# hmorimitsu/ptlflow

Measured on AMD Instinct MI355X. Metric: frame-pairs/sec, RAFT 32-iter 436x1024, higher is better.
Workload: dtype f32; 1 GPU; raft random-init (seeded), 436x1024 frame pairs, 32 iterations, fp32, batch 8/GPU, eval forward incl. encoders, mask head + convex upsample on every iteration as the reference; global_batch=8, parallelism=dp1 (independent replicas, no collectives)

## Files before the change

ptlflow_amd/csrc/pfk_wino.hip:

```cpp
#include "pfk_gemm.h"

using namespace pfkg;

namespace {

constexpr int WT = 32;
constexpr int WN = 64;
constexpr int WK = 8;
constexpr int UIMG = 16 * WN * WK;

typedef float f32x2 __attribute__((ext_vector_type(2)));
typedef __attribute__((address_space(3))) float lfloat;
typedef __attribute__((address_space(3))) f32x2 lf32x2;
typedef __attribute__((address_space(3))) f32x4 lf32x4;

struct WinoArgs {
  const float* src; int ld;
  unsigned src_bytes;
  int H, W;
  int tw, tpi;
  int ntiles;
  int nks;
  const float* weight; unsigned w_bytes;
  const float* bias;
  int cout;
  int ncb;
  int relu; float scale;
  float* out; int out_ld, out_coff;
  unsigned out_bytes;
  const float* res; int res_ld;
  unsigned res_bytes;
  int relu2;
  int vec;
  const float* in_mean; const float* in_rstd;
  unsigned stat_bytes;
  int cin, in_relu;
  int nbi;
  double* part; long long astride;
};

constexpr unsigned T_OK = 0x80000000u, T_ROW2 = 0x40000000u, T_COL2 = 0x20000000u, T_PIX = 0x1fffffffu;
constexpr int ESZ = 64 * 32 + 4 * 16;

__device__ __forceinline__ __amdgpu_buffer_rsrc_t rsrc_n(const void* p, unsigned bytes) {
  return __builtin_amdgcn_make_buffer_rsrc(const_cast<void*>(p), 0, (int)bytes, 0x00020000);
}

__device__ __forceinline__ void wino_load_stat(__amdgpu_buffer_rsrc_t rm, __amdgpu_buffer_rsrc_t rr, unsigned soff, int ks, float (&mr)[2]) {
  mr[0] = __builtin_bit_cast(float, __builtin_amdgcn_raw_buffer_load_b32(rm, soff, ks * WK * 4, 0));
  mr[1] = __builtin_bit_cast(float, __builtin_amdgcn_raw_buffer_load_b32(rr, soff, ks * WK * 4, 0));
}

__device__ __forceinline__ void wino_load_v2(__amdgpu_buffer_rsrc_t rs, const unsigned (&voff)[16], int ks, int q, float (&d)[16]) {
  d[q] = __builtin_bit_cast(float, __builtin_amdgcn_raw_buffer_load_b32(rs, voff[q], ks * WK * 4, 0));
  d[q + 1] = __builtin_bit_cast(float, __builtin_amdgcn_raw_buffer_load_b32(rs, voff[q + 1], ks * WK * 4, 0));
}

__device__ __forceinline__ void wino_dma_u(__amdgpu_buffer_rsrc_t rw, lfloat* dst, unsigned wvoff, unsigned wk, int j) {
#if defined(__HIP_DEVICE_COMPILE__)
  __builtin_amdgcn_raw_ptr_buffer_load_lds(rw, (__attribute__((address_space(3))) void*)(dst + j * 1024), 16, wvoff, wk + j * 4096u, 0, 0);
#endif
}

template <bool NORM>
__device__ __forceinline__ void wino_mfma(const lfloat* aV, const lfloat* aU, const lfloat* aU1, f32x4 (&acc)[16][2], bool more,
                                          __amdgpu_buffer_rsrc_t rw, lfloat* udst, unsigned wvoff, unsigned wk,
                                          __amdgpu_buffer_rsrc_t rs, const unsigned (&voff)[16], int ks, float (&d)[16],
                                          __amdgpu_buffer_rsrc_t rm, __amdgpu_buffer_rsrc_t rr, unsigned soff, float (&mr)[2]) {
  f32x2 va[2], u0[2], u1[2];
  va[0] = *(const lf32x2*)(aV);
  u0[0] = *(const lf32x2*)(aU);
  u1[0] = *(const lf32x2*)(aU1);
  __builtin_amdgcn_sched_barrier(0);
#pragma unroll
  for (int x = 0; x < 16; ++x) {
    const int c = x & 1, n = c ^ 1;
    if (x + 1 < 16) {
      va[n] = *(const lf32x2*)(aV + (x + 1) * WT * WK);
      u0[n] = *(const lf32x2*)(aU + (x + 1) * WN * WK);
      u1[n] = *(const lf32x2*)(aU1 + (x + 1) * WN * WK);
    }
    if (more) {
      if (x < 8) wino_dma_u(rw, udst, wvoff, wk, x);
      else wino_load_v2(rs, voff, ks, 2 * (x - 8), d);
      if constexpr (NORM) {
        if (x == 8) wino_load_stat(rm, rr, soff, ks, mr);
      }
    }
    __builtin_amdgcn_sched_barrier(0);
    acc[x][0] = __builtin_amdgcn_mfma_f32_16x16x4f32(va[c][0], u0[c][0], acc[x][0], 0, 0, 0);
    acc[x][1] = __builtin_amdgcn_mfma_f32_16x16x4f32(va[c][0], u1[c][0], acc[x][1], 0, 0, 0);
    acc[x][0] = __builtin_amdgcn_mfma_f32_16x16x4f32(va[c][1], u0[c][1], acc[x][0], 0, 0, 0);
    acc[x][1] = __builtin_amdgcn_mfma_f32_16x16x4f32(va[c][1], u1[c][1], acc[x][1], 0, 0, 0);
    __builtin_amdgcn_sched_barrier(0);
  }
}

typedef __attribute__((address_space(3))) unsigned lunsigned;
typedef unsigned int u32x4v __attribute__((__vector_size__(16)));

template <bool RES, bool VEC>
__device__ __forceinline__ void wino_epi_request(const WinoArgs& a, const lunsigned* tT, int n0, unsigned (&oo)[8], f32x4 (&r4)[8]) {
  unsigned ro[8];
#pragma unroll
  for (int i = 0; i < 8; ++i) {
    oo[i] = tT[2 * i] + (unsigned)(a.out_coff + n0) * 4u;
    if constexpr (RES) ro[i] = tT[4 * WT + 2 * i] + (unsigned)n0 * 4u;
  }
  if constexpr (RES) {
    const __amdgpu_buffer_rsrc_t rr = rsrc_n(a.res, a.res_bytes);
#pragma unroll
    for (int i = 0; i < 8; ++i) {
      if constexpr (VEC) {
        r4[i] = __builtin_bit_cast(f32x4, __builtin_amdgcn_raw_buffer_load_b128(rr, ro[i], 0, 0));
      } else {
#pragma unroll
        for (int j = 0; j < 4; ++j)
          r4[i][j] = __builtin_bit_cast(float, __builtin_amdgcn_raw_buffer_load_b32(rr, n0 + j < a.cout ? ro[i] + 4u * j : OOB, 0, 0));
      }
    }
  }
}

template <bool RES, bool VEC, bool STATS>
__device__ __forceinline__ void wino_epi_store(const WinoArgs& a, const lfloat* rE, int n0, const unsigned (&oo)[8], const f32x4 (&r4)[8],
                                               double (&st)[8]) {
  const __amdgpu_buffer_rsrc_t ro = rsrc_n(a.out, a.out_bytes);
  const __amdgpu_buffer_rsrc_t rbias = rsrc_n(a.bias, a.bias != nullptr ? (unsigned)a.cout * 4u : 0u);
  float bias4[4];
#pragma unroll
  for (int j = 0; j < 4; ++j) bias4[j] = __builtin_bit_cast(float, __builtin_amdgcn_raw_buffer_load_b32(rbias, (unsigned)(n0 + j) * 4u, 0, 0));
  const float lo = a.relu ? 0.f : -__builtin_inff(), lo2 = a.relu2 ? 0.f : -__builtin_inff();
#pragma unroll
  for (int i = 0; i < 8; ++i) {
    const f32x4 y = *(const lf32x4*)(rE + i * 256 + (i >> 1) * 16);
    float v[4];
#pragma unroll
    for (int j = 0; j < 4; ++j) {
      float t = y[j] + bias4[j];
      t = (t < lo) ? lo : t;
      if constexpr (RES) {
        t = __builtin_fmaf(t, a.scale, r4[i][j]);
        t = (t < lo2) ? lo2 : t;
      } else {
        t *= a.scale;
      }
      v[j] = t;
      if constexpr (STATS) {
        const double dv = (double)((oo[i] < OOB && (VEC || n0 + j < a.cout)) ? t : 0.f);
        st[j] += dv;
        st[4 + j] = __builtin_fma(dv, dv, st[4 + j]);
      }
    }
    if constexpr (VEC) {
      __builtin_amdgcn_raw_buffer_store_b128(__builtin_bit_cast(u32x4v, (f32x4{v[0], v[1], v[2], v[3]})), ro, oo[i], 0, 0);
    } else {
#pragma unroll
      for (int j = 0; j < 4; ++j)
        __builtin_amdgcn_raw_buffer_store_b32(__builtin_bit_cast(unsigned, v[j]), ro, n0 + j < a.cout ? oo[i] + 4u * j : OOB, 0, 0);
    }
  }
}

template <bool RES, bool NORM = false, bool STATS = false>
__global__ __launch_bounds__(256, 2) void conv_gemm_wino_f32_kernel(const WinoArgs a) {
  static_assert(!(RES && STATS), "the residual form is never in front of an instance norm");
  __shared__ __attribute__((aligned(16))) float smem[2 * UIMG + 16 * WT * WK];
  lfloat* const sU = (lfloat*)smem;
  lfloat* const sV = sU + 2 * UIMG;

  const int tid = threadIdx.x, lane = tid & 63, wid = __builtin_amdgcn_readfirstlane(tid >> 6);
  const int cb = blockIdx.x % a.ncb;
  const int t0 = (blockIdx.x / a.ncb) * WT;

  const __amdgpu_buffer_rsrc_t rs = rsrc_n(a.src, a.src_bytes);
  const __amdgpu_buffer_rsrc_t rw = rsrc_n(a.weight, a.w_bytes);
  const __amdgpu_buffer_rsrc_t rm = rsrc_n(a.in_mean, NORM ? a.stat_bytes : 0u);
  const __amdgpu_buffer_rsrc_t rr = rsrc_n(a.in_rstd, NORM ? a.stat_bytes : 0u);

  const int lt = tid >> 3, cc = tid & 7;
  unsigned voff[16];
  unsigned tinfo;
  unsigned soff = 0;
  {
    int g, b, r;
    bool tok;
    if constexpr (STATS) {
      const int tb = blockIdx.x / a.ncb;
      b = tb / a.nbi;
      r = (tb - b * a.nbi) * WT + lt;
      tok = r < a.tpi;
    } else {
      g = t0 + lt;
      tok = g < a.ntiles;
      b = g / a.tpi;
      r = g - b * a.tpi;
    }
    if constexpr (NORM) soff = ((unsigned)b * (unsigned)a.cin + (unsigned)cc) * 4u;
    const int ty = r / a.tw, tx = r - ty * a.tw;
    tinfo = tok ? (T_OK | (2 * ty + 1 < a.H ? T_ROW2 : 0u) | (2 * tx + 1 < a.W ? T_COL2 : 0u) | (unsigned)((b * a.H + 2 * ty) * a.W + 2 * tx)) : 0u;
#pragma unroll
    for (int i = 0; i < 4; ++i)
#pragma unroll
      for (int j = 0; j < 4; ++j) {
        const int y = 2 * ty - 1 + i, x = 2 * tx - 1 + j;
        const bool ok = tok && (unsigned)y < (unsigned)a.H && (unsigned)x < (unsigned)a.W;
        voff[i * 4 + j] = ok ? ((unsigned)((b * a.H + y) * a.W + x) * (unsigned)a.ld + (unsigned)cc) * 4u : OOB;
      }
  }
  const int vslot = ((cc & 3) * 2 + (cc >> 2)) ^ (((lt >> 2) & 3) * 2);
  lfloat* const vdst = sV + lt * WK + vslot;
  const unsigned wvoff = (unsigned)lane * 16u;
  const unsigned wbase = (unsigned)cb * (unsigned)a.nks * (UIMG * 4u) + (unsigned)wid * 1024u;
  lfloat* const udst = sU + wid * 256;

  float d[16];
  float mr[2] = {0.f, 0.f};
  const int wt = wid & 1, wc = wid >> 1;
  const int rl = lane & 15, kq = lane >> 4;
  const lfloat* const aV = sV + (wt * 16 + rl) * WK + ((kq * 2) ^ (((rl >> 2) & 3) * 2));
  const lfloat* const aU = sU + (wc * 32 + rl) * WK + ((kq * 2) ^ (((rl >> 2) & 3) * 2));
  const lfloat* aU1 = aU + 16 * WK;
  asm volatile("" : "+v"(aU1));

  f32x4 acc[16][2];
#pragma unroll
  for (int x = 0; x < 16; ++x)
#pragma unroll
    for (int c = 0; c < 2; ++c) acc[x][c] = f32x4{0.f, 0.f, 0.f, 0.f};

#pragma unroll
  for (int j = 0; j < 8; ++j) {
    wino_dma_u(rw, udst, wvoff, wbase, j);
    wino_load_v2(rs, voff, 0, 2 * j, d);
  }
  if constexpr (NORM) wino_load_stat(rm, rr, soff, 0, mr);
  const float nlo = a.in_relu ? 0.f : -__builtin_inff();  for (int ks = 0; ks < a.nks; ++ks) {
    if constexpr (NORM) {
#pragma unroll
      for (int q = 0; q < 16; ++q) {
        const float y = __fmul_rn(__fsub_rn(d[q], mr[0]), mr[1]);
        d[q] = voff[q] == OOB ? 0.f : ((y < nlo) ? nlo : y);
      }
    }
    float t[16];
#pragma unroll
    for (int j = 0; j < 4; ++j) {
      t[0 * 4 + j] = d[0 * 4 + j] - d[2 * 4 + j];
      t[1 * 4 + j] = d[1 * 4 + j] + d[2 * 4 + j];
      t[2 * 4 + j] = d[2 * 4 + j] - d[1 * 4 + j];
      t[3 * 4 + j] = d[1 * 4 + j] - d[3 * 4 + j];
    }
#pragma unroll
    for (int i = 0; i < 4; ++i) {
      vdst[(i * 4 + 0) * WT * WK] = t[i * 4 + 0] - t[i * 4 + 2];
      vdst[(i * 4 + 1) * WT * WK] = t[i * 4 + 1] + t[i * 4 + 2];
      vdst[(i * 4 + 2) * WT * WK] = t[i * 4 + 2] - t[i * 4 + 1];
      vdst[(i * 4 + 3) * WT * WK] = t[i * 4 + 1] - t[i * 4 + 3];
    }
    asm volatile("s_waitcnt vmcnt(0) lgkmcnt(0)\n\ts_barrier" ::: "memory");
    const int ub = (ks & 1) * UIMG;
    wino_mfma<NORM>(aV, aU + ub, aU1 + ub, acc, ks + 1 < a.nks, rw, udst + (UIMG - ub), wvoff, wbase + (unsigned)(ks + 1) * (UIMG * 4u),
                    rs, voff, ks + 1, d, rm, rr, soff, mr);
    asm volatile("s_waitcnt lgkmcnt(0)\n\ts_barrier" ::: "memory");
  }

  lfloat* const sE = (lfloat*)smem + wid * ESZ;
  lunsigned* const sT = (lunsigned*)((lfloat*)smem + 4 * ESZ);
  static_assert(4 * ESZ + 8 * WT <= 2 * UIMG + 16 * WT * WK, "parking areas and offset table must fit into the loop's LDS");
  {
    const unsigned need = T_OK | ((cc & 2) ? T_ROW2 : 0u) | ((cc & 1) ? T_COL2 : 0u);
    const bool ok = (tinfo & need) == need;
    const unsigned pix = (tinfo & T_PIX) + (unsigned)(((cc >> 1) & 1) * a.W + (cc & 1));
    const unsigned po = ok ? pix * (unsigned)a.out_ld * 4u : OOB;
    const unsigned pr = ok ? pix * (unsigned)a.res_ld * 4u : OOB;
    if (cc < 4) {
      sT[cc * WT + lt] = po;
      if constexpr (RES) sT[(4 + cc) * WT + lt] = pr;
    }
  }
  asm volatile("s_waitcnt lgkmcnt(0)\n\ts_barrier" ::: "memory");

  const int prow = lane >> 3, c4 = (lane & 7) * 4;
  const int n0 = cb * WN + wc * 32 + c4;
  const lunsigned* const tT = sT + (prow & 3) * WT + wt * 16 + (lane >> 5);
  const bool vec = a.vec && cb * WN + wc * 32 + 32 <= a.cout;
  unsigned oo[8];
  f32x4 r4[8];
  if (vec) wino_epi_request<RES, true>(a, tT, n0, oo, r4);
  else wino_epi_request<RES, false>(a, tT, n0, oo, r4);

  {
    lfloat* const pE = sE + kq * (16 * 32 + 16) + rl;
#pragma unroll
    for (int c = 0; c < 2; ++c)
#pragma unroll
      for (int r = 0; r < 4; ++r) {
        float m[16];
#pragma unroll
        for (int x = 0; x < 16; ++x) m[x] = acc[x][c][r];
        float s0[4], s1[4];
#pragma unroll
        for (int j = 0; j < 4; ++j) {
          s0[j] = m[0 * 4 + j] + m[1 * 4 + j] + m[2 * 4 + j];
          s1[j] = m[1 * 4 + j] - m[2 * 4 + j] - m[3 * 4 + j];
        }
        pE[(r * 4 + 0) * 32 + c * 16] = s0[0] + s0[1] + s0[2];
        pE[(r * 4 + 1) * 32 + c * 16] = s0[1] - s0[2] - s0[3];
        pE[(r * 4 + 2) * 32 + c * 16] = s1[0] + s1[1] + s1[2];
        pE[(r * 4 + 3) * 32 + c * 16] = s1[1] - s1[2] - s1[3];
      }
  }
  const lfloat* const rE = sE + prow * 32 + c4;
  double st[8] = {0., 0., 0., 0., 0., 0., 0., 0.};
  if (vec) wino_epi_store<RES, true, STATS>(a, rE, n0, oo, r4, st);
  else wino_epi_store<RES, false, STATS>(a, rE, n0, oo, r4, st);

  if constexpr (STATS) {
    typedef __attribute__((address_space(3))) double ldouble;
    ldouble* const sS = (ldouble*)(sE) + lane * 8;
#pragma unroll
    for (int j = 0; j < 8; ++j) sS[j] = st[j];
    asm volatile("s_waitcnt lgkmcnt(0)\n\ts_barrier" ::: "memory");
    if (tid < 2 * WN) {
      const int which = tid >> 6, col = tid & 63;
      const int idx = ((col & 31) >> 2) * 8 + which * 4 + (col & 3);
      double tot[2];
#pragma unroll
      for (int w = 0; w < 2; ++w) {
        const ldouble* const p = (const ldouble*)((lfloat*)smem + ((col >> 5) * 2 + w) * ESZ) + idx;
        double s = 0.;
#pragma unroll
        for (int k = 0; k < 8; ++k) s += p[k * 64];
        tot[w] = s;
      }
      const int n = cb * WN + col;
      if (n < a.cout) a.part[which * a.astride + (long long)(blockIdx.x / a.ncb) * a.cout + n] = tot[0] + tot[1];
    }
  }
}

constexpr int WN1 = 128;
constexpr int VIMG1 = 8 * WT * WK;

struct Wino1dArgs {
  const float* src0; const float* src1;
  int ld0, ld1;
  unsigned bytes0, bytes1;
  int nks0, nks;
  int H, W;
  int L, nt;
  int ntiles;
  const float* weight; unsigned w_bytes;
  const float* bias;
  int cout, ncb;
  int relu; float scale;
  float* out; int out_ld, out_coff;
  const float* res; int res_ld;
  float* h; int h_ld;
  float* aux_z; float* aux_rh;
  int ch;
};

template <bool VERT>
__device__ __forceinline__ void wino1d_tile(const Wino1dArgs& a, int g, int& base, int& t) {
  if constexpr (VERT) {
    const int r = g / a.W, x = g - r * a.W, b = r / a.nt;
    t = r - b * a.nt;
    base = b * a.H * a.W + x;
  } else {
    const int line = g / a.nt;
    t = g - line * a.nt;
    base = line * a.W;
  }
}

__device__ __forceinline__ void wino1d_load_v(__amdgpu_buffer_rsrc_t rs0, __amdgpu_buffer_rsrc_t rs1, const unsigned (&voff0)[8],
                                              const unsigned (&voff1)[8], bool s1, int soff, int q, float (&d)[8]) {
  d[q] = s1 ? __builtin_bit_cast(float, __builtin_amdgcn_raw_buffer_load_b32(rs1, voff1[q], soff, 0))
            : __builtin_bit_cast(float, __builtin_amdgcn_raw_buffer_load_b32(rs0, voff0[q], soff, 0));
}

__device__ __forceinline__ void wino1d_mfma(const lfloat* aV, const lfloat* aU0, const lfloat* aU1, const lfloat* aU2, const lfloat* aU3,
                                            f32x4 (&acc)[8][4], bool more, __amdgpu_buffer_rsrc_t rw, lfloat* udst, unsigned wvoff,
                                            unsigned wk, __amdgpu_buffer_rsrc_t rs0, __amdgpu_buffer_rsrc_t rs1,
                                            const unsigned (&voff0)[8], const unsigned (&voff1)[8], bool s1, int soff, float (&d)[8]) {
  f32x2 va[2], u[2][4];
  va[0] = *(const lf32x2*)(aV);
  u[0][0] = *(const lf32x2*)(aU0);
  u[0][1] = *(const lf32x2*)(aU1);
  u[0][2] = *(const lf32x2*)(aU2);
  u[0][3] = *(const lf32x2*)(aU3);
  __builtin_amdgcn_sched_barrier(0);
#pragma unroll
  for (int x = 0; x < 8; ++x) {
    const int c = x & 1, n = c ^ 1;
    if (x + 1 < 8) {
      va[n] = *(const lf32x2*)(aV + (x + 1) * WT * WK);
      u[n][0] = *(const lf32x2*)(aU0 + (x + 1) * WN1 * WK);
      u[n][1] = *(const lf32x2*)(aU1 + (x + 1) * WN1 * WK);
      u[n][2] = *(const lf32x2*)(aU2 + (x + 1) * WN1 * WK);
      u[n][3] = *(const lf32x2*)(aU3 + (x + 1) * WN1 * WK);
    }
    if (more) {
      wino_dma_u(rw, udst, wvoff, wk, x);
      wino1d_load_v(rs0, rs1, voff0, voff1, s1, soff, x, d);
    }
    __builtin_amdgcn_sched_barrier(0);
#pragma unroll
    for (int s = 0; s < 2; ++s)
#pragma unroll
      for (int f = 0; f < 4; ++f) acc[x][f] = __builtin_amdgcn_mfma_f32_16x16x4f32(va[c][s], u[c][f][s], acc[x][f], 0, 0, 0);
    __builtin_amdgcn_sched_barrier(0);
  }
}

__device__ __forceinline__ void wino1d_at(const f32x4 (&acc)[8][4], int f, int r, float (&y)[4]) {
  const float p12 = acc[1][f][r] + acc[2][f][r], q12 = acc[1][f][r] - acc[2][f][r];
  const float p34 = acc[3][f][r] + acc[4][f][r], q34 = acc[3][f][r] - acc[4][f][r];
  const float p56 = acc[5][f][r] + acc[6][f][r], q56 = acc[5][f][r] - acc[6][f][r];
  y[0] = acc[0][f][r] + p12 + p34 + p56;
  y[1] = q12 + 2.f * q34 + 0.5f * q56;
  y[2] = p12 + 4.f * p34 + 0.25f * p56;
  y[3] = q12 + 8.f * q34 + 0.125f * q56 + acc[7][f][r];
}

template <bool VERT, int EPI>
__global__ __launch_bounds__(256, 2) void conv_gemm_wino1d_f32_kernel(const Wino1dArgs a) {
  __shared__ __attribute__((aligned(16))) float smem[2 * UIMG + VIMG1];
  lfloat* const sU = (lfloat*)smem;
  lfloat* const sV = sU + 2 * UIMG;

  const int tid = threadIdx.x, lane = tid & 63, wid = __builtin_amdgcn_readfirstlane(tid >> 6);
  const int cb = blockIdx.x % a.ncb;
  const int t0 = (blockIdx.x / a.ncb) * WT;
  const int pstride = VERT ? a.W : 1;

  const __amdgpu_buffer_rsrc_t rs0 = rsrc_n(a.src0, a.bytes0);
  const __amdgpu_buffer_rsrc_t rs1 = rsrc_n(a.src1, a.bytes1);
  const __amdgpu_buffer_rsrc_t rw = rsrc_n(a.weight, a.w_bytes);

  const int lt = tid >> 3, cc = tid & 7;
  unsigned voff0[8], voff1[8];
  {
    const int g = t0 + lt;
    const bool tok = g < a.ntiles;
    int base, t;
    wino1d_tile<VERT>(a, g, base, t);
#pragma unroll
    for (int j = 0; j < 8; ++j) {
      const int ax = 4 * t - 2 + j;
      const bool ok = tok && (unsigned)ax < (unsigned)a.L;
      const unsigned pix = (unsigned)(base + ax * pstride);
      voff0[j] = ok ? (pix * (unsigned)a.ld0 + (unsigned)cc) * 4u : OOB;
      voff1[j] = ok ? (pix * (unsigned)a.ld1 + (unsigned)cc) * 4u : OOB;
    }
  }
  const int vslot = ((cc & 3) * 2 + (cc >> 2)) ^ (((lt >> 2) & 3) * 2);
  lfloat* const vdst = sV + lt * WK + vslot;
  const unsigned wvoff = (unsigned)lane * 16u;
  const unsigned wbase = (unsigned)cb * (unsigned)a.nks * (UIMG * 4u) + (unsigned)wid * 1024u;
  lfloat* const udst = sU + wid * 256;

  float d[8];
  const int wt = wid & 1, wc = wid >> 1;
  const int rl = lane & 15, kq = lane >> 4;
  const int oslot = (kq * 2) ^ (((rl >> 2) & 3) * 2);
  const lfloat* const aV = sV + (wt * 16 + rl) * WK + oslot;
  const lfloat* const aU0 = sU + (wc * 64 + rl) * WK + oslot;
  const lfloat* aU1 = aU0 + 16 * WK;
  const lfloat* aU2 = aU0 + 32 * WK;
  const lfloat* aU3 = aU0 + 48 * WK;
  asm volatile("" : "+v"(aU1));
  asm volatile("" : "+v"(aU2));
  asm volatile("" : "+v"(aU3));

  f32x4 acc[8][4];
#pragma unroll
  for (int x = 0; x < 8; ++x)
#pragma unroll
    for (int f = 0; f < 4; ++f) acc[x][f] = f32x4{0.f, 0.f, 0.f, 0.f};

#pragma unroll
  for (int j = 0; j < 8; ++j) {
    wino_dma_u(rw, udst, wvoff, wbase, j);
    wino1d_load_v(rs0, rs1, voff0, voff1, false, 0, j, d);
  }
  for (int ks = 0; ks < a.nks; ++ks) {
    {
      const float e12 = d[2] - 4.25f * d[4] + d[6], o12 = d[1] - 4.25f * d[3] + d[5];
      const float e34 = 0.25f * d[2] - 1.25f * d[4] + d[6], o34 = 0.5f * d[1] - 2.5f * d[3] + 2.f * d[5];
      const float e56 = 4.f * d[2] - 5.f * d[4] + d[6], o56 = 2.f * d[1] - 2.5f * d[3] + 0.5f * d[5];
      vdst[0 * WT * WK] = (d[6] - d[0]) + 5.25f * (d[2] - d[4]);
      vdst[1 * WT * WK] = e12 + o12;
      vdst[2 * WT * WK] = e12 - o12;
      vdst[3 * WT * WK] = e34 + o34;
      vdst[4 * WT * WK] = e34 - o34;
      vdst[5 * WT * WK] = e56 + o56;
      vdst[6 * WT * WK] = e56 - o56;
      vdst[7 * WT * WK] = (d[7] - d[1]) + 5.25f * (d[3] - d[5]);
    }
    asm volatile("s_waitcnt vmcnt(0) lgkmcnt(0)\n\ts_barrier" ::: "memory");
    const int ub = (ks & 1) * UIMG;
    const int kn = ks + 1;
    const bool s1 = kn >= a.nks0;
    const int soff = (kn - (s1 ? a.nks0 : 0)) * WK * 4;
    wino1d_mfma(aV, aU0 + ub, aU1 + ub, aU2 + ub, aU3 + ub, acc, kn < a.nks, rw, udst + (UIMG - ub), wvoff,
                wbase + (unsigned)kn * (UIMG * 4u), rs0, rs1, voff0, voff1, s1, soff, d);
    asm volatile("s_waitcnt lgkmcnt(0)\n\ts_barrier" ::: "memory");
  }

  typedef __attribute__((address_space(1))) float gfloat;
  if constexpr (EPI == PFK_EPI_LINEAR) {
#pragma unroll
    for (int f = 0; f < 4; ++f) {
      const int n = cb * WN1 + wc * 64 + f * 16 + rl;
      const bool nok = n < a.cout;
      const float bias = (a.bias != nullptr && nok) ? a.bias[n] : 0.f;
#pragma unroll
      for (int r = 0; r < 4; ++r) {
        const int g = t0 + wt * 16 + kq * 4 + r;
        float y[4];
        wino1d_at(acc, f, r, y);
        if (!nok || g >= a.ntiles) continue;
        int base, t;
        wino1d_tile<VERT>(a, g, base, t);
#pragma unroll
        for (int e = 0; e < 4; ++e) {
          const int ax = 4 * t + e;
          if (ax >= a.L) continue;
          const long long p = base + ax * pstride;
          float v = y[e] + bias;
          if (a.relu) v = (v < 0.f) ? 0.f : v;
          v *= a.scale;
          ((gfloat*)a.out)[p * a.out_ld + a.out_coff + n] = v;
        }
      }
    }
  } else {
    constexpr int ES = 68;
    static_assert(4 * 64 * ES <= 2 * UIMG + VIMG1, "the four waves' parking areas must fit into the loop's LDS");
    lfloat* const sE = (lfloat*)smem + wid * (64 * ES);
#pragma unroll
    for (int f = 0; f < 4; ++f)
#pragma unroll
      for (int r = 0; r < 4; ++r) {
        float y[4];
        wino1d_at(acc, f, r, y);
#pragma unroll
        for (int e = 0; e < 4; ++e) sE[((kq * 4 + r) * 4 + e) * ES + f * 16 + rl] = y[e];
      }
    const int prow = lane >> 4, col4 = (lane & 15) * 4;
    const int n0 = cb * WN1 + wc * 64 + col4;
    const bool nok = n0 < a.cout;
    const int nc = nok ? n0 : 0;
    const int ch = a.ch;
    f32x4 bias4 = f32x4{0.f, 0.f, 0.f, 0.f};
    if (a.bias != nullptr) bias4 = f32x4{a.bias[nc], a.bias[nc + 1], a.bias[nc + 2], a.bias[nc + 3]};
    const bool upper = nc >= ch;
    const int hc = (EPI == PFK_EPI_GRU_ZR) ? (upper ? nc - ch : 0) : nc;
#pragma unroll
    for (int half = 0; half < 2; ++half) {
      bool ok[8];
      long long p[8];
      f32x4 r4[8], h4[8], z4[8];
#pragma unroll
      for (int i = 0; i < 8; ++i) {
        const int li = (half * 8 + i) * 4 + prow;
        const int g = t0 + wt * 16 + (li >> 2);
        int base, t;
        wino1d_tile<VERT>(a, g, base, t);
        const int ax = 4 * t + (li & 3);
        ok[i] = nok && g < a.ntiles && ax < a.L;
        p[i] = ok[i] ? base + ax * pstride : 0;
        r4[i] = f32x4{0.f, 0.f, 0.f, 0.f};
        if (a.res != nullptr) r4[i] = *(const f32x4*)(a.res + p[i] * a.res_ld + nc);
        if constexpr (EPI == PFK_EPI_GRU_ZR) {
          if (upper) h4[i] = *(const f32x4*)(a.h + p[i] * a.h_ld + hc);
        } else {
          z4[i] = *(const f32x4*)(a.aux_z + p[i] * ch + nc);
          h4[i] = *(const f32x4*)(a.h + p[i] * a.h_ld + hc);
        }
      }
#pragma unroll
      for (int i = 0; i < 8; ++i) {
        const int li = (half * 8 + i) * 4 + prow;
        const f32x4 v = *(const lf32x4*)(sE + li * ES + col4) + bias4 + r4[i];
        f32x4 o;
        if constexpr (EPI == PFK_EPI_GRU_ZR) {
#pragma unroll
          for (int e = 0; e < 4; ++e) o[e] = sigmoid_f(v[e]);
          if (!ok[i]) continue;
          if (upper) {
#pragma unroll
            for (int e = 0; e < 4; ++e) o[e] *= h4[i][e];
            *(f32x4*)(a.aux_rh + p[i] * ch + hc) = o;
          } else {
            *(f32x4*)(a.aux_z + p[i] * ch + nc) = o;
          }
        } else {
#pragma unroll
          for (int e = 0; e < 4; ++e) {
            const float keep = __fmul_rn(__fsub_rn(1.0f, z4[i][e]), h4[i][e]);
            const float take = __fmul_rn(z4[i][e], tanhf(v[e]));
            o[e] = __fadd_rn(keep, take);
          }
          if (!ok[i]) continue;
          *(f32x4*)(a.h + p[i] * a.h_ld + hc) = o;
        }
      }
    }
  }
}

template <bool VERT>
static void wino1d_launch_epi(const Wino1dArgs& a, int epilogue, unsigned nblk, hipStream_t st) {
  switch (epilogue) {
    case PFK_EPI_GRU_ZR: hipLaunchKernelGGL((conv_gemm_wino1d_f32_kernel<VERT, PFK_EPI_GRU_ZR>), dim3(nblk), dim3(256), 0, st, a); break;
    case PFK_EPI_GRU_Q: hipLaunchKernelGGL((conv_gemm_wino1d_f32_kernel<VERT, PFK_EPI_GRU_Q>), dim3(nblk), dim3(256), 0, st, a); break;
    default: hipLaunchKernelGGL((conv_gemm_wino1d_f32_kernel<VERT, PFK_EPI_LINEAR>), dim3(nblk), dim3(256), 0, st, a); break;
  }
}

}

extern "C" {

long long pfk_conv_wino1d_weight_floats(int ktot, int cout) {
  if (ktot <= 0 || cout <= 0 || (ktot & 7)) return PFK_ERR_BAD_ARG;
  return 8LL * ktot * ((cout + WN1 - 1) / WN1 * WN1);
}

int pfk_conv1d_wino_f32(const pfk_conv_desc* d, pfk_stream_t stream) {
  if (!d) return PFK_ERR_BAD_ARG;
  const bool vert = d->kh == 5 && d->kw == 1;
  if (!vert && !(d->kh == 1 && d->kw == 5)) return PFK_ERR_UNSUPPORTED;
  if (d->stride > 1 || d->num_src < 1 || d->num_src > 2 || d->relu_after_residual) return PFK_ERR_UNSUPPORTED;
  if (d->epilogue != PFK_EPI_LINEAR && d->epilogue != PFK_EPI_GRU_ZR && d->epilogue != PFK_EPI_GRU_Q) return PFK_ERR_UNSUPPORTED;
  if (d->cout_active > 0 && d->cout_active < d->cout) return PFK_ERR_UNSUPPORTED;
  if (d->epilogue == PFK_EPI_LINEAR && d->residual) return PFK_ERR_UNSUPPORTED;
  if (!d->weight || d->B <= 0 || d->H <= 0 || d->W <= 0 || d->cout <= 0) return PFK_ERR_BAD_ARG;
  const long long M = (long long)d->B * d->H * d->W;
  int ktot = 0;
  for (int i = 0; i < d->num_src; ++i) {
    const pfk_conv_src& s = d->src[i];
    if (!s.ptr || s.channels <= 0 || s.ld < s.channels) return PFK_ERR_BAD_ARG;
    if (s.channels & 7) return PFK_ERR_UNSUPPORTED;
    if (reinterpret_cast<uintptr_t>(s.ptr) & 3u) return PFK_ERR_ALIGNMENT;
    if (M * s.ld * 4 >= 0x7fffffffLL) return PFK_ERR_UNSUPPORTED;
    ktot += s.channels;
  }
  const int ch = d->epilogue == PFK_EPI_GRU_ZR ? d->cout / 2 : d->cout;
  if (d->epilogue == PFK_EPI_LINEAR) {
    if (!d->out || d->out_coff < 0 || d->out_ld < d->out_coff + d->cout) return PFK_ERR_BAD_ARG;
    if (reinterpret_cast<uintptr_t>(d->out) & 3u) return PFK_ERR_ALIGNMENT;
  } else {
    if (!d->h || !d->aux_z || d->h_ld < ch || (d->epilogue == PFK_EPI_GRU_ZR && (!d->aux_rh || (d->cout & 1))) || (ch & 3))
      return PFK_ERR_BAD_ARG;
    if (d->residual && d->residual_ld < d->cout) return PFK_ERR_BAD_ARG;
    if (!pfk_aligned16(d->h) || !pfk_aligned16(d->aux_z) || !pfk_aligned16(d->aux_rh) || !pfk_aligned16(d->residual) || (d->h_ld & 3) ||
        (d->residual && (d->residual_ld & 3)))
      return PFK_ERR_ALIGNMENT;
  }
  if (!pfk_aligned16(d->weight)) return PFK_ERR_ALIGNMENT;
  const long long wfloats = pfk_conv_wino1d_weight_floats(ktot, d->cout);
  if (wfloats * 4 >= 0x7fffffffLL) return PFK_ERR_UNSUPPORTED;
  Wino1dArgs a{};
  const pfk_conv_src& s0 = d->src[0];
  const pfk_conv_src& s1 = d->src[d->num_src - 1];
  a.src0 = s0.ptr; a.ld0 = s0.ld; a.bytes0 = (unsigned)(((M - 1) * s0.ld + s0.channels) * 4);
  a.src1 = s1.ptr; a.ld1 = s1.ld; a.bytes1 = (unsigned)(((M - 1) * s1.ld + s1.channels) * 4);
  a.nks0 = s0.channels / WK; a.nks = ktot / WK;
  a.H = d->H; a.W = d->W;
  a.L = vert ? d->H : d->W;
  a.nt = (a.L + 3) / 4;
  const long long ntiles = (long long)d->B * (vert ? d->W : d->H) * a.nt;
  a.ncb = (d->cout + WN1 - 1) / WN1;
  const long long nblk = (ntiles + WT - 1) / WT * a.ncb;
  if (nblk >= 0x7fffffffLL) return PFK_ERR_UNSUPPORTED;
  a.ntiles = (int)ntiles;
  a.weight = d->weight; a.w_bytes = (unsigned)(wfloats * 4);
  a.bias = d->bias;
  a.cout = d->cout;
  a.relu = d->relu ? 1 : 0; a.scale = d->scale;
  a.out = d->out; a.out_ld = d->out_ld; a.out_coff = d->out_coff;
  a.res = d->residual; a.res_ld = d->residual_ld;
  a.h = d->h; a.h_ld = d->h_ld; a.aux_z = d->aux_z; a.aux_rh = d->aux_rh; a.ch = ch;
  if (vert) wino1d_launch_epi<true>(a, d->epilogue, (unsigned)nblk, static_cast<hipStream_t>(stream));
  else wino1d_launch_epi<false>(a, d->epilogue, (unsigned)nblk, static_cast<hipStream_t>(stream));
  return pfk_launch_status();
}

long long pfk_conv_wino_weight_floats(int cin, int cout) {
  if (cin <= 0 || cout <= 0 || (cin & 31)) return PFK_ERR_BAD_ARG;
  return 16LL * cin * ((cout + WN - 1) / WN * WN);
}

static inline long long wino_blocks_per_image(int H, int W) { return ((long long)((H + 1) / 2) * ((W + 1) / 2) + WT - 1) / WT; }

struct WinoFuse {
  bool norm, stats;
  const float* in_mean; const float* in_rstd; int in_relu;
  float eps; float* out_mean; float* out_rstd; void* workspace; long long workspace_bytes;
};

static int wino_launch(const pfk_conv_desc* d, bool res, pfk_stream_t stream, const WinoFuse* f = nullptr) {
  if (!d) return PFK_ERR_BAD_ARG;
  const bool norm = f && f->norm, stats = f && f->stats;
  if (norm && (!f->in_mean || !f->in_rstd)) return PFK_ERR_BAD_ARG;
  if (stats && (!f->out_mean || !f->out_rstd || !f->workspace || d->residual || d->relu_after_residual)) return PFK_ERR_BAD_ARG;
  if (d->num_src != 1 || d->kh != 3 || d->kw != 3 || d->stride > 1 || d->epilogue != PFK_EPI_LINEAR)
    return PFK_ERR_UNSUPPORTED;
  if (!res && (d->residual || d->relu_after_residual)) return PFK_ERR_UNSUPPORTED;
  if (res && (!d->residual || d->residual_ld < d->cout || (reinterpret_cast<uintptr_t>(d->residual) & 3u))) return PFK_ERR_BAD_ARG;
  const pfk_conv_src& s = d->src[0];
  if (!s.ptr || !d->weight || !d->out || d->B <= 0 || d->H <= 0 || d->W <= 0 || d->cout <= 0 || s.channels <= 0 ||
      s.ld < s.channels || d->out_coff < 0 || d->out_ld < d->out_coff + d->cout)
    return PFK_ERR_BAD_ARG;
  if (s.channels & 31) return PFK_ERR_UNSUPPORTED;
  if (!pfk_aligned16(d->weight) || (reinterpret_cast<uintptr_t>(s.ptr) & 3u) || (reinterpret_cast<uintptr_t>(d->out) & 3u))
    return PFK_ERR_ALIGNMENT;
  const long long M = (long long)d->B * d->H * d->W;
  const long long src_bytes = ((M - 1) * s.ld + s.channels) * 4;
  const long long wfloats = pfk_conv_wino_weight_floats(s.channels, d->cout);
  if (M * s.ld * 4 >= 0x7fffffffLL || wfloats * 4 >= 0x7fffffffLL) return PFK_ERR_UNSUPPORTED;
  const long long out_bytes = ((M - 1) * d->out_ld + d->out_coff + d->cout) * 4;
  const long long res_bytes = res ? ((M - 1) * d->residual_ld + d->cout) * 4 : 0;
  if (out_bytes >= 0x7fffffffLL || res_bytes >= 0x7fffffffLL) return PFK_ERR_UNSUPPORTED;
  int ncb = (d->cout + WN - 1) / WN;
  if (d->cout_active > 0 && d->cout_active < d->cout) {
    if (d->cout_active & (WN - 1)) return PFK_ERR_UNSUPPORTED;
    ncb = d->cout_active / WN;
    if (stats) return PFK_ERR_UNSUPPORTED;
  }
  if (norm && ((reinterpret_cast<uintptr_t>(f->in_mean) | reinterpret_cast<uintptr_t>(f->in_rstd)) & 3u)) return PFK_ERR_ALIGNMENT;
  if (stats) {
    if (reinterpret_cast<uintptr_t>(f->workspace) & 7u) return PFK_ERR_ALIGNMENT;
    if (f->workspace_bytes < pfk_conv_wino_stats_workspace_bytes(d->B, d->H, d->W, d->cout)) return PFK_ERR_BAD_ARG;
  }
  WinoArgs a{};
  a.src = s.ptr; a.ld = s.ld; a.src_bytes = (unsigned)src_bytes;
  a.H = d->H; a.W = d->W;
  a.tw = (d->W + 1) / 2;
  a.tpi = a.tw * ((d->H + 1) / 2);
  const long long ntiles = (long long)d->B * a.tpi;
  const long long nbi = wino_blocks_per_image(d->H, d->W);
  const long long nblk = (stats ? d->B * nbi : (ntiles + WT - 1) / WT) * ncb;
  if (nblk >= 0x7fffffffLL || ntiles >= 0x7fffffffLL) return PFK_ERR_UNSUPPORTED;
  a.ntiles = (int)ntiles;
  a.nks = s.channels / WK;
  a.weight = d->weight; a.w_bytes = (unsigned)(wfloats * 4);
  a.bias = d->bias;
  a.cout = d->cout;
  a.ncb = ncb;
  a.relu = d->relu ? 1 : 0; a.scale = d->scale;
  a.out = d->out; a.out_ld = d->out_ld; a.out_coff = d->out_coff; a.out_bytes = (unsigned)out_bytes;
  a.vec = pfk_aligned16(d->out + d->out_coff) && !(d->out_ld & 3) && (!res || (pfk_aligned16(d->residual) && !(d->residual_ld & 3)));
  if (norm) {
    a.in_mean = f->in_mean; a.in_rstd = f->in_rstd; a.in_relu = f->in_relu ? 1 : 0;
    a.cin = s.channels; a.stat_bytes = (unsigned)((long long)d->B * s.channels * 4);
  }
  hipStream_t st = static_cast<hipStream_t>(stream);
  if (stats) {
    a.nbi = (int)nbi;
    a.part = static_cast<double*>(f->workspace);
    a.astride = (long long)d->B * nbi * d->cout;
    if (norm) hipLaunchKernelGGL((conv_gemm_wino_f32_kernel<false, true, true>), dim3((unsigned)nblk), dim3(256), 0, st, a);
    else hipLaunchKernelGGL((conv_gemm_wino_f32_kernel<false, false, true>), dim3((unsigned)nblk), dim3(256), 0, st, a);
    return pfk_instnorm_finish_parts(a.part, d->B, a.nbi, d->cout, d->H * d->W, f->eps, f->out_mean, f->out_rstd, st);
  }
  if (norm) {
    if (res) return PFK_ERR_UNSUPPORTED;
    hipLaunchKernelGGL((conv_gemm_wino_f32_kernel<false, true, false>), dim3((unsigned)nblk), dim3(256), 0, st, a);
    return pfk_launch_status();
  }
  if (res) {
    if (d->cout_active > 0 && d->cout_active < d->cout) return PFK_ERR_UNSUPPORTED;
    a.res = d->residual; a.res_ld = d->residual_ld; a.res_bytes = (unsigned)res_bytes; a.relu2 = d->relu_after_residual ? 1 : 0;
    hipLaunchKernelGGL(conv_gemm_wino_f32_kernel<true>, dim3((unsigned)nblk), dim3(256), 0, static_cast<hipStream_t>(stream), a);
  } else {
    hipLaunchKernelGGL(conv_gemm_wino_f32_kernel<false>, dim3((unsigned)nblk), dim3(256), 0, static_cast<hipStream_t>(stream), a);
  }
  return pfk_launch_status();
}

int pfk_conv2d_wino_f32(const pfk_conv_desc* d, pfk_stream_t stream) { return wino_launch(d, false, stream); }

int pfk_conv2d_wino_res_f32(const pfk_conv_desc* d, pfk_stream_t stream) { return wino_launch(d, true, stream); }

int pfk_conv2d_wino_norm_f32(const pfk_conv_desc* d, const float* in_mean, const float* in_rstd, int in_relu, pfk_stream_t stream) {
  const WinoFuse f{true, false, in_mean, in_rstd, in_relu, 0.f, nullptr, nullptr, nullptr, 0};
  return wino_launch(d, false, stream, &f);
}

long long pfk_conv_wino_stats_workspace_bytes(int B, int H, int W, int cout) {
  if (B <= 0 || H <= 0 || W <= 0 || cout <= 0) return PFK_ERR_BAD_ARG;
  return 2LL * B * wino_blocks_per_image(H, W) * cout * (long long)sizeof(double);
}

int pfk_conv2d_wino_stats_f32(const pfk_conv_desc* d, const float* in_mean, const float* in_rstd, int in_relu, float eps,
                              float* out_mean, float* out_rstd, void* workspace, long long workspace_bytes, pfk_stream_t stream) {
  if ((in_mean == nullptr) != (in_rstd == nullptr)) return PFK_ERR_BAD_ARG;
  const WinoFuse f{in_mean != nullptr, true, in_mean, in_rstd, in_relu, eps, out_mean, out_rstd, workspace, workspace_bytes};
  return wino_launch(d, false, stream, &f);
}


}
```

Measured before the change: 125.0 frame-pairs/s.

## Software-pipeline 1D Winograd conv: double-buffer V tile, prefetch input two K-steps ahead

Restructures the 1D Winograd conv main loop so the input transform for the next K-step runs inside the MFMA loop into a second V buffer. Global input loads are issued two steps ahead, with a partial vmcnt wait. This removes the serial transform-then-barrier phase before each MFMA block and leaves a single barrier per step. The cost is extra LDS for the second V image, possibly lowering occupancy, plus more register pressure from holding two input vectors.

```diff
diff --git a/ptlflow_amd/csrc/pfk_wino.hip b/ptlflow_amd/csrc/pfk_wino.hip
--- a/ptlflow_amd/csrc/pfk_wino.hip
+++ b/ptlflow_amd/csrc/pfk_wino.hip
@@ -381,11 +381,36 @@
             : __builtin_bit_cast(float, __builtin_amdgcn_raw_buffer_load_b32(rs0, voff0[q], soff, 0));
 }
 
-__device__ __forceinline__ void wino1d_mfma(const lfloat* aV, const lfloat* aU0, const lfloat* aU1, const lfloat* aU2, const lfloat* aU3,
-                                            f32x4 (&acc)[8][4], bool more, __amdgpu_buffer_rsrc_t rw, lfloat* udst, unsigned wvoff,
-                                            unsigned wk, __amdgpu_buffer_rsrc_t rs0, __amdgpu_buffer_rsrc_t rs1,
-                                            const unsigned (&voff0)[8], const unsigned (&voff1)[8], bool s1, int soff, float (&d)[8]) {
+__device__ __forceinline__ void wino1d_bt(const float (&d)[8], float (&v)[8]) {
+  const float e12 = d[2] - 4.25f * d[4] + d[6], o12 = d[1] - 4.25f * d[3] + d[5];
+  const float e34 = 0.25f * d[2] - 1.25f * d[4] + d[6], o34 = 0.5f * d[1] - 2.5f * d[3] + 2.f * d[5];
+  const float e56 = 4.f * d[2] - 5.f * d[4] + d[6], o56 = 2.f * d[1] - 2.5f * d[3] + 0.5f * d[5];
+  v[0] = (d[6] - d[0]) + 5.25f * (d[2] - d[4]);
+  v[1] = e12 + o12;
+  v[2] = e12 - o12;
+  v[3] = e34 + o34;
+  v[4] = e34 - o34;
+  v[5] = e56 + o56;
+  v[6] = e56 - o56;
+  v[7] = (d[7] - d[1]) + 5.25f * (d[3] - d[5]);
+}
+
+template <bool MORE, bool MORE2>
+__device__ __forceinline__ void wino1d_step(int ks, int nks0, const lfloat* aV, const lfloat* aU0, const lfloat* aU1, const lfloat* aU2,
+                                            const lfloat* aU3, f32x4 (&acc)[8][4], __amdgpu_buffer_rsrc_t rw, lfloat* udst,
+                                            unsigned wvoff, unsigned wbase, lfloat* vdst, __amdgpu_buffer_rsrc_t rs0,
+                                            __amdgpu_buffer_rsrc_t rs1, const unsigned (&voff0)[8], const unsigned (&voff1)[8],
+                                            float (&d)[8]) {
+  const int ub = (ks & 1) * UIMG, vb = (ks & 1) * VIMG1;
+  const int k2 = ks + 2;
+  const bool s1 = k2 >= nks0;
+  const int soff = (k2 - (s1 ? nks0 : 0)) * WK * 4;
+  const unsigned wk = wbase + (unsigned)(ks + 1) * (UIMG * 4u);
+  lfloat* const vnext = vdst + (VIMG1 - vb);
+  udst += UIMG - ub;
+  aV += vb; aU0 += ub; aU1 += ub; aU2 += ub; aU3 += ub;
   f32x2 va[2], u[2][4];
+  float v[8];
   va[0] = *(const lf32x2*)(aV);
   u[0][0] = *(const lf32x2*)(aU0);
   u[0][1] = *(const lf32x2*)(aU1);
@@ -402,9 +427,24 @@
       u[n][2] = *(const lf32x2*)(aU2 + (x + 1) * WN1 * WK);
       u[n][3] = *(const lf32x2*)(aU3 + (x + 1) * WN1 * WK);
     }
-    if (more) {
-      wino_dma_u(rw, udst, wvoff, wk, x);
-      wino1d_load_v(rs0, rs1, voff0, voff1, s1, soff, x, d);
+    if constexpr (MORE) {
+      if (x == 1) {
+        wino1d_bt(d, v);
+#pragma unroll
+        for (int j = 0; j < 8; ++j) vnext[j * WT * WK] = v[j];
+        __builtin_amdgcn_sched_barrier(0);
+      }
+      if (x >= 1 && x <= 4) {
+        wino_dma_u(rw, udst, wvoff, wk, 2 * (x - 1));
+        wino_dma_u(rw, udst, wvoff, wk, 2 * (x - 1) + 1);
+      }
+    }
+    if constexpr (MORE2) {
+      if (x >= 4) {
+        __builtin_amdgcn_sched_barrier(0);
+        wino1d_load_v(rs0, rs1, voff0, voff1, s1, soff, 2 * (x - 4), d);
+        wino1d_load_v(rs0, rs1, voff0, voff1, s1, soff, 2 * (x - 4) + 1, d);
+      }
     }
     __builtin_amdgcn_sched_barrier(0);
 #pragma unroll
@@ -413,6 +453,8 @@
       for (int f = 0; f < 4; ++f) acc[x][f] = __builtin_amdgcn_mfma_f32_16x16x4f32(va[c][s], u[c][f][s], acc[x][f], 0, 0, 0);
     __builtin_amdgcn_sched_barrier(0);
   }
+  if constexpr (MORE2) asm volatile("s_waitcnt vmcnt(8) lgkmcnt(0)\n\ts_barrier" ::: "memory");
+  else asm volatile("s_waitcnt vmcnt(0) lgkmcnt(0)\n\ts_barrier" ::: "memory");
 }
 
 __device__ __forceinline__ void wino1d_at(const f32x4 (&acc)[8][4], int f, int r, float (&y)[4]) {
@@ -427,7 +469,7 @@
 
 template <bool VERT, int EPI>
 __global__ __launch_bounds__(256, 2) void conv_gemm_wino1d_f32_kernel(const Wino1dArgs a) {
-  __shared__ __attribute__((aligned(16))) float smem[2 * UIMG + VIMG1];
+  __shared__ __attribute__((aligned(16))) float smem[2 * UIMG + 2 * VIMG1];
   lfloat* const sU = (lfloat*)smem;
   lfloat* const sV = sU + 2 * UIMG;
 
@@ -462,7 +504,7 @@
   const unsigned wbase = (unsigned)cb * (unsigned)a.nks * (UIMG * 4u) + (unsigned)wid * 1024u;
   lfloat* const udst = sU + wid * 256;
 
-  float d[8];
+  float d[8] = {0.f, 0.f, 0.f, 0.f, 0.f, 0.f, 0.f, 0.f};
   const int wt = wid & 1, wc = wid >> 1;
   const int rl = lane & 15, kq = lane >> 4;
   const int oslot = (kq * 2) ^ (((rl >> 2) & 3) * 2);
@@ -481,34 +523,34 @@
 #pragma unroll
     for (int f = 0; f < 4; ++f) acc[x][f] = f32x4{0.f, 0.f, 0.f, 0.f};
 
-#pragma unroll
-  for (int j = 0; j < 8; ++j) {
-    wino_dma_u(rw, udst, wvoff, wbase, j);
-    wino1d_load_v(rs0, rs1, voff0, voff1, false, 0, j, d);
-  }
-  for (int ks = 0; ks < a.nks; ++ks) {
-    {
-      const float e12 = d[2] - 4.25f * d[4] + d[6], o12 = d[1] - 4.25f * d[3] + d[5];
-      const float e34 = 0.25f * d[2] - 1.25f * d[4] + d[6], o34 = 0.5f * d[1] - 2.5f * d[3] + 2.f * d[5];
-      const float e56 = 4.f * d[2] - 5.f * d[4] + d[6], o56 = 2.f * d[1] - 2.5f * d[3] + 0.5f * d[5];
-      vdst[0 * WT * WK] = (d[6] - d[0]) + 5.25f * (d[2] - d[4]);
-      vdst[1 * WT * WK] = e12 + o12;
-      vdst[2 * WT * WK] = e12 - o12;
-      vdst[3 * WT * WK] = e34 + o34;
-      vdst[4 * WT * WK] = e34 - o34;
-      vdst[5 * WT * WK] = e56 + o56;
-      vdst[6 * WT * WK] = e56 - o56;
-      vdst[7 * WT * WK] = (d[7] - d[1]) + 5.25f * (d[3] - d[5]);
-    }
-    asm volatile("s_waitcnt vmcnt(0) lgkmcnt(0)\n\ts_barrier" ::: "memory");
-    const int ub = (ks & 1) * UIMG;
-    const int kn = ks + 1;
-    const bool s1 = kn >= a.nks0;
-    const int soff = (kn - (s1 ? a.nks0 : 0)) * WK * 4;
-    wino1d_mfma(aV, aU0 + ub, aU1 + ub, aU2 + ub, aU3 + ub, acc, kn < a.nks, rw, udst + (UIMG - ub), wvoff,
-                wbase + (unsigned)kn * (UIMG * 4u), rs0, rs1, voff0, voff1, s1, soff, d);
-    asm volatile("s_waitcnt lgkmcnt(0)\n\ts_barrier" ::: "memory");
-  }
+  {
+    float d0[8], v[8];
+#pragma unroll
+    for (int j = 0; j < 8; ++j) wino1d_load_v(rs0, rs1, voff0, voff1, false, 0, j, d0);
+#pragma unroll
+    for (int j = 0; j < 8; ++j) wino_dma_u(rw, udst, wvoff, wbase, j);
+    __builtin_amdgcn_sched_barrier(0);
+    if (a.nks > 1) {
+      const bool s1 = 1 >= a.nks0;
+      const int soff = (1 - (s1 ? a.nks0 : 0)) * WK * 4;
+#pragma unroll
+      for (int j = 0; j < 8; ++j) wino1d_load_v(rs0, rs1, voff0, voff1, s1, soff, j, d);
+    }
+    __builtin_amdgcn_sched_barrier(0);
+    wino1d_bt(d0, v);
+#pragma unroll
+    for (int j = 0; j < 8; ++j) vdst[j * WT * WK] = v[j];
+  }
+  if (a.nks > 1) asm volatile("s_waitcnt vmcnt(8) lgkmcnt(0)\n\ts_barrier" ::: "memory");
+  else asm volatile("s_waitcnt vmcnt(0) lgkmcnt(0)\n\ts_barrier" ::: "memory");
+  int ks = 0;
+  for (; ks + 2 < a.nks; ++ks)
+    wino1d_step<true, true>(ks, a.nks0, aV, aU0, aU1, aU2, aU3, acc, rw, udst, wvoff, wbase, vdst, rs0, rs1, voff0, voff1, d);
+  if (ks + 1 < a.nks) {
+    wino1d_step<true, false>(ks, a.nks0, aV, aU0, aU1, aU2, aU3, acc, rw, udst, wvoff, wbase, vdst, rs0, rs1, voff0, voff1, d);
+    ++ks;
+  }
+  wino1d_step<false, false>(ks, a.nks0, aV, aU0, aU1, aU2, aU3, acc, rw, udst, wvoff, wbase, vdst, rs0, rs1, voff0, voff1, d);
 
   typedef __attribute__((address_space(1))) float gfloat;
   if constexpr (EPI == PFK_EPI_LINEAR) {
```

New measurement: 125.8 frame-pairs/s (median of 6 runs). Within noise of the previous version (+0.6%).
